# tahaspc82442/federated_multi_modal

Measured on AMD Instinct MI355X. Metric: images/sec/node (ViT-B/16 MaPLe fwd+bwd), higher is better.
Workload: dtype fp16; 1 GPU; c4: PatternNet-shape 38-class synthetic, J=9, batch=32 per client (configs[3]); clients=1, batch_per_client=32, global_batch=32, classes=38, prompt_depth=9, n_ctx=2, parallelism=one federated client per GPU x1, FedAvg all-reduce per round, round=512 local steps + 1 FedAvg, hipgraph=True

## Files before the change

### federated_multi_modal_amd/_lib.py

```python
from __future__ import annotations

import ctypes
import os
from pathlib import Path

_HERE = Path(__file__).resolve().parent
LIB_PATH = _HERE / "lib" / "libmapfed.so"

P, I, L, F = ctypes.c_void_p, ctypes.c_int, ctypes.c_int64, ctypes.c_float

SIGNATURES = {
    "mf_abi_version": [],
    "mf_gemm_nt": [P, L, P, L, P, L, I, I, I, P, P, P, L, I, I, P],
    "mf_gemm": [P, L, I, P, L, I, P, L, I, I, I, P, P, P, L, I, I, P],
    "mf_layernorm_fwd": [P, L, P, P, P, P, L, P, P, I, I, P],
    "mf_layernorm_bwd_blocks": [I],
    "mf_layernorm_bwd": [P, L, P, L, P, P, P, P, P, L, P, L, P, P, P, I, I, I, P],
    "mf_col_reduce_desc_bytes": [],
    "mf_col_reduce_batch": [P, I, I, P],
    "mf_attention_fwd": [P, L, P, L, P, I, I, I, I, I, P],
    "mf_attention_fwd_rows": [P, L, P, L, P, I, I, I, I, I, I, P],
    "mf_attention_bwd": [P, L, P, L, P, L, P, P, I, P, L, I, I, I, I, P],
    "mf_attention_bwd_rows": [P, L, P, L, P, L, P, I, P, L, I, I, I, I, I, P],
    "mf_qkv_attention_fwd": [P, L, I, P, P, P, L, P, L, P, I, I, I, I, I, P],
# ... 6 lines not shown
    "mf_transpose_f16": [P, L, P, L, I, I, P],
    "mf_colsum_blocks": [I],
    "mf_colsum_f16": [P, L, I, I, P, I, P, P],
    "mf_cast_f16_f32": [P, P, L, P],
    "mf_small_linear_fwd": [P, P, P, P, I, I, I, I, P],
    "mf_small_linear_bwd": [P, P, P, P, P, P, I, I, I, I, I, P],
    "mf_gemm_splitk_ws_floats": [I, I, I, I],
    "mf_small_linear_desc_bytes": [],
    "mf_small_linear_fwd_batch": [P, I, I, P],
    "mf_small_linear_bwd_batch": [P, I, I, I, I, P],
    "mf_clip_head_fwd": [P, P, I, I, I, P, P, P, P, P, P, P],
    "mf_clip_loss_fwd_bwd": [P, P, P, P, P, P, P, I, I, I, P, P, P, P, P, P, P, P, P],
    "mf_layernorm_bwd_inject": [P, L, P, L, P, P, P, P, L, P, L, P, I, I, P, I, I, I, P],
    "mf_layernorm_fwd_inject": [P, L, P, P, P, L, P, P, I, I, P, I, I, I, P],
    "mf_gemm_splitk": [P, L, I, P, L, I, P, L, I, I, I, P, L, I, I, P],
    "mf_clip_loss_soft_fwd_bwd": [P, P, P, P, P, P, P, I, I, I, P, P, P, P, P, P, P, P, P, P],
    "mf_argmax_correct": [P, I, I, P, P, P, P],
    "mf_optim_chunk_bytes": [],
    "mf_optim_chunk_elems": [],
    "mf_clip_grad_norm": [P, P, P, I, F, P, P, P],
    "mf_sgd_step": [P, P, P, L, I, P, P, P],
    "mf_optimizer_step": [P, P, P, L, P, P, P, L, P, I, F, P, P, P, P, P, P],
    "mf_sgd_prox_step": [P, P, P, P, L, I, P, P, P],
    "mf_optimizer_step_prox": [P, P, P, L, P, P, P, L, P, I, F, P, P, P, P, P, P, P, P],
    "mf_fedavg_pack_weighted": [P, L, P, L, P, F, P, P],
    "mf_fedavg_unpack_weighted": [P, P, L, P, L, P, P, P],
    "mf_fedavg_pack": [P, L, P, L, P, P, P],
    "mf_fedavg_unpack": [P, P, L, P, L, P, P, P],
    "mf_fedopt_step": [P, I, I, F, F, F, F, P, P, P, P, L, P, L, P, P, P],
    "mf_fedopt_deliver": [P, P, L, P, L, P, P, P],
# ... 55 lines not shown
```

### federated_multi_modal_amd/csrc/elementwise.hip

```cpp
#include "mf_common.h"

namespace {

template <typename TIn>
__global__ void im2col_kernel(const TIn* __restrict__ img, f16* __restrict__ out, int B, int R, int P) {
  const int G = R / P;
  const int K = 3 * P * P;
  const int chunks_per_row = K / 8;
  const int64_t t = (int64_t)blockIdx.x * blockDim.x + threadIdx.x;
  const int64_t total = (int64_t)B * G * G * chunks_per_row;
  if (t >= total) return;
  const int ch = t % chunks_per_row;
  const int64_t prow = t / chunks_per_row;
  const int b = prow / (G * G), pp = prow % (G * G);
  const int py = pp / G, px = pp % G;
  const int k = ch * 8;
  const int c = k / (P * P), kh = (k / P) % P, kw = k % P;
  const TIn* src = img + (((int64_t)b * 3 + c) * R + (py * P + kh)) * R + px * P + kw;
  f16x8 v;
  if constexpr (sizeof(TIn) == 4) {
    const f32x4 a = *(const f32x4*)src, d = *(const f32x4*)(src + 4);
#pragma unroll
    for (int e = 0; e < 4; ++e) {
      v[e] = (f16)a[e];
// ... 203 lines not shown
    return;
  }
  const int tx = t & 63, ty = t >> 6;
  for (int i = ty; i < 64; i += 4) {
    const int r = r0 + i, c = c0 + tx;
    tile[i][tx] = (r < R && c < C) ? in[(int64_t)r * ld_in + c] : (f16)0.f;
  }
  __syncthreads();
  for (int i = ty; i < 64; i += 4) {
    const int c = c0 + i, r = r0 + tx;
    if (c < C && r < R) out[(int64_t)c * ld_out + r] = tile[tx][i];
  }
}

constexpr int CS_ROWS = 64;
__global__ __launch_bounds__(256) void colsum_part_kernel(const f16* __restrict__ in, int64_t ld, int R, int C,
                                                          float* __restrict__ part) {
  __shared__ f32x4 red[4][64];
  const int lane = threadIdx.x & 63, w = threadIdx.x >> 6;
  const int c = blockIdx.x * 256 + lane * 4;
  const int r0 = blockIdx.y * CS_ROWS + w * 16;
  f32x4 s = {0.f, 0.f, 0.f, 0.f};
  if (c < C) {
#pragma unroll 4
    for (int r = r0; r < min(R, r0 + 16); ++r) {
      f16x4 v = *(const f16x4*)(in + (int64_t)r * ld + c);
#pragma unroll
      for (int e = 0; e < 4; ++e) s[e] += (float)v[e];
    }
  }
  red[w][lane] = s;
  __syncthreads();
  if (w == 0 && c < C) {
    f32x4 t = red[0][lane];
#pragma unroll
// ... 266 lines not shown
  MF_CHECK_LAUNCH();
  return 0;
}

extern "C" int mf_transpose_f16(const void* in, int64_t ld_in, void* out, int64_t ld_out, int R, int C,
                                void* stream) {
  if (R <= 0 || C <= 0) return 0;
  dim3 grid((C + 63) / 64, (R + 63) / 64);
  transpose_kernel<<<grid, 256, 0, (hipStream_t)stream>>>((const f16*)in, ld_in, (f16*)out, ld_out, R, C);
  MF_CHECK_LAUNCH();
  return 0;
}

extern "C" int mf_colsum_blocks(int R) { return (R + CS_ROWS - 1) / CS_ROWS; }

extern "C" int mf_colsum_f16(const void* in, int64_t ld, int R, int C, void* out, int out_f16, float* workspace,
                             void* stream) {
  if (R <= 0 || C <= 0) return 0;
  const int nb = mf_colsum_blocks(R);
  hipStream_t st = (hipStream_t)stream;
  if (C % 4 || ld % 4) return mf_set_error("mf_colsum_f16: C and ld must be multiples of 4", -1);
  dim3 grid((C + 255) / 256, nb);
  colsum_part_kernel<<<grid, 256, 0, st>>>((const f16*)in, ld, R, C, workspace);
  MF_CHECK_LAUNCH();
  if (out_f16)
    col_reduce_kernel<true><<<dim3((C + 63) / 64, 1), 1024, 0, st>>>(workspace, workspace, nb, C, C, out, out, 0);
  else
    col_reduce_kernel<false><<<dim3((C + 63) / 64, 1), 1024, 0, st>>>(workspace, workspace, nb, C, C, out, out, 0);
  MF_CHECK_LAUNCH();
  return 0;
}

extern "C" int mf_small_linear_fwd(const void* X, const void* W, const void* b, void* Y, int M, int I, int O,
                                   int is_f16, void* stream) {
  if (M <= 0) return 0;
  hipStream_t st = (hipStream_t)stream;
  const int64_t threads = (int64_t)M * O * 64;
  if (is_f16)
    small_linear_fwd_kernel<f16><<<nblk(threads), 256, 0, st>>>((const f16*)X, (const f16*)W, (const f16*)b, (f16*)Y,
                                                               M, I, O);
  else
    small_linear_fwd_kernel<float><<<nblk(threads), 256, 0, st>>>((const float*)X, (const float*)W,
                                                                  (const float*)b, (float*)Y, M, I, O);
  MF_CHECK_LAUNCH();
  return 0;
// ... 76 lines not shown
```

### federated_multi_modal_amd/csrc/gemm.hip

```cpp
#include <algorithm>
#include <cstdlib>
#include <type_traits>

#include "mf_common.h"

namespace {

enum Epi : int {
  EPI_NONE = 0,
  EPI_BIAS = 1,
  EPI_BIAS_RESID = 2,
  EPI_BIAS_GELU = 3,
  EPI_DGELU = 4,
  EPI_F32 = 5,
  EPI_RESID = 6,
};

struct GemmArgs {
  const f16* A;
  const f16* B;
  void* C;
  const f16* bias;
  const f16* aux_in;
  f16* aux_out;
  int64_t lda, ldb, ldc, ld_aux;
  int M, N, K;
  int vec8;
  int ksplit;
  int xb;
};

MF_DEV void st16_stream(f16* p, f16x8 v) { __builtin_nontemporal_store(v, (f16x8*)p); }

MF_DEV void tile_of(int p, int tiles_m, int tiles_n, int xb, int& mt, int& nt) {
  const int nb = 1 << xb, ma = 8 >> xb;
  int off = 0;
#pragma unroll 1
  for (int x = 0; x < 8; ++x) {
    const int ia = x >> xb, jb = x & (nb - 1);
    const int m_lo = tiles_m * ia / ma, m_hi = tiles_m * (ia + 1) / ma;
    const int n_lo = tiles_n * jb / nb, n_hi = tiles_n * (jb + 1) / nb;
    const int sz = (m_hi - m_lo) * (n_hi - n_lo);
    if (p < off + sz) {
      const int loc = p - off, w = n_hi - n_lo;
// ... 226 lines not shown
}

template <int A_INS, int B_INS>
MF_DEV void dma_stage(const f16* A, int a_bytes, const f16* B, int b_bytes, f16* la, f16* lb,
                      const int* a_voff, const int* a_dst, const int* b_voff, const int* b_dst, int a_k, int b_k) {
  const auto a_rsrc = __builtin_amdgcn_make_buffer_rsrc((void*)A, 0, a_bytes, 0x00020000);
  const auto b_rsrc = __builtin_amdgcn_make_buffer_rsrc((void*)B, 0, b_bytes, 0x00020000);
#pragma unroll
  for (int i = 0; i < A_INS; ++i)
    __builtin_amdgcn_raw_ptr_buffer_load_lds(a_rsrc, (lds_ptr_t)(la + a_dst[i]), 16, a_voff[i] + a_k, 0, 0, 0);
#pragma unroll
  for (int i = 0; i < B_INS; ++i)
    __builtin_amdgcn_raw_ptr_buffer_load_lds(b_rsrc, (lds_ptr_t)(lb + b_dst[i]), 16, b_voff[i] + b_k, 0, 0, 0);
}

template <int BM, int BN, int WM, int WN, int S, int EPI, bool TA = false, bool TB = false>
__global__ __launch_bounds__(WM * WN * 64) void gemm_nt_kernel(GemmArgs g0) {
  GemmArgs g = g0;
  constexpr int NW = WM * WN;
  constexpr int NT = NW * 64;
  constexpr int WTM = BM / WM, WTN = BN / WN;
  constexpr int TM = WTM / 16, TN = WTN / 16;
  constexpr int A_INS = BM / 8 / NW;
  constexpr int B_INS = BN / 8 / NW;
  static_assert(A_INS * 8 * NW == BM && B_INS * 8 * NW == BN, "tile / wave split");
  static_assert((!TA || BM == 64 || BM == 128) && (!TB || BN == 64 || BN == 128), "K-major image widths");
  constexpr int STAGE = (BM + BN) * BK;
  constexpr int LDS_ELEMS = S * STAGE > BM * (BN + 8) ? S * STAGE : BM * (BN + 8);
  __shared__ __attribute__((aligned(1024))) f16 lds[LDS_ELEMS];

  const int tid = threadIdx.x;
  const int lane = tid & 63;
  const int wid = __builtin_amdgcn_readfirstlane(tid >> 6);
  const int wave_m = wid / WN, wave_n = wid % WN;

  const int tiles_n = (g.N + BN - 1) / BN;
  const int tiles_m = (g.M + BM - 1) / BM;
  const bool legacy = g.ksplit > 0 && g.xb == 2;
  const int nwg = legacy ? tiles_m * tiles_n : gridDim.x;
  const int bid = legacy ? blockIdx.x % nwg : blockIdx.x;
  const int xcd = bid & 7, q = nwg >> 3, r = nwg & 7;
  const int wgid = (xcd < r ? xcd * (q + 1) : r * (q + 1) + (xcd - r) * q) + (bid >> 3);
  int mt, nt;
  if (g.ksplit > 0) {
    int z;
    if (legacy) {
      z = blockIdx.x / nwg;
      tile_of(wgid, tiles_m, tiles_n, 0, mt, nt);
    } else {
      split_tile_of(wgid, tiles_m, tiles_n, g.xb != 0, z, mt, nt);
    }
    const int k0 = z * g.ksplit;
    g.A += (int64_t)k0 * (TA ? g.lda : 1);
    g.B += (int64_t)k0 * (TB ? g.ldb : 1);
    g.K = min(g.ksplit, g.K - k0);
    g.C = (float*)g.C + (int64_t)z * g.M * g.ldc;
  } else {
    tile_of(wgid, tiles_m, tiles_n, g.xb, mt, nt);
  }
  const int m0 = mt * BM;
  const int n0 = nt * BN;

  const int a_bytes = (int)((TA ? (int64_t)(g.K - 1) * g.lda + g.M : (int64_t)(g.M - 1) * g.lda + g.K) * 2);
  const int b_bytes = (int)((TB ? (int64_t)(g.K - 1) * g.ldb + g.N : (int64_t)(g.N - 1) * g.ldb + g.K) * 2);
  int a_voff[A_INS], a_dst[A_INS], b_voff[B_INS], b_dst[B_INS];
#pragma unroll
  for (int i = 0; i < A_INS; ++i) dma_setup<TA, BM>(lane, wid, g.lda, m0, i, A_INS, a_voff[i], a_dst[i]);
// ... 2 lines not shown
  const int a_kstep = TA ? (int)(g.lda * 2) : 2, b_kstep = TB ? (int)(g.ldb * 2) : 2;
#define MF_STAGE(buf, k0)                                                                                     \
  dma_stage<A_INS, B_INS>(g.A, a_bytes, g.B, b_bytes, lds + (buf)*STAGE, lds + (buf)*STAGE + BM * BK, a_voff, a_dst, \
                          b_voff, b_dst, (k0)*a_kstep, (k0)*b_kstep)



  f32x4 acc[TM][TN];
#pragma unroll
  for (int i = 0; i < TM; ++i)
#pragma unroll
    for (int j = 0; j < TN; ++j) acc[i][j] = (f32x4){0.f, 0.f, 0.f, 0.f};

  MF_STAMP(0);
  const int nk = (g.K + BK - 1) / BK;
#pragma unroll
  for (int p = 0; p < S - 1; ++p)
    if (p < nk) MF_STAGE(p, p * BK);

  const int fr = lane & 15, fg = lane >> 4;
  for (int kt = 0; kt < nk; ++kt) {
    const int younger = min(S - 2, nk - 1 - kt);
    if constexpr (S >= 3) {
      if (younger >= 2) wait_vmcnt<2 * (A_INS + B_INS)>();
      else if (younger == 1) wait_vmcnt<A_INS + B_INS>();
      else wait_vmcnt<0>();
    } else {
      wait_vmcnt<0>();
    }
    __builtin_amdgcn_s_barrier();
    if (kt == 0) MF_STAMP(1);
    if (kt + S - 1 < nk) MF_STAGE((kt + S - 1) % S, (kt + S - 1) * BK);
    const f16* la = lds + (kt % S) * STAGE;
    const f16* lb = la + BM * BK;
    f16x8 af[2][TM], bf[2][TN];
#pragma unroll
    for (int s = 0; s < 2; ++s) {
#pragma unroll
      for (int i = 0; i < TM; ++i) {
        const int row = wave_m * WTM + i * 16 + fr;
        if constexpr (TA)
          af[s][i] = frag_t<BM>(la, 32 * s + 8 * fg, wave_m * WTM + i * 16, fr);
        else
          af[s][i] = *(const f16x8*)(la + row * BK + swz(row, 4 * s + fg) * 8);
      }
#pragma unroll
      for (int j = 0; j < TN; ++j) {
        const int row = wave_n * WTN + j * 16 + fr;
        if constexpr (TB)
          bf[s][j] = frag_t<BN>(lb, 32 * s + 8 * fg, wave_n * WTN + j * 16, fr);
        else
          bf[s][j] = *(const f16x8*)(lb + row * BK + swz(row, 4 * s + fg) * 8);
      }
    }
#pragma unroll
    for (int s = 0; s < 2; ++s)
#pragma unroll
      for (int i = 0; i < TM; ++i)
#pragma unroll
        for (int j = 0; j < TN; ++j)
          acc[i][j] = __builtin_amdgcn_mfma_f32_16x16x32_f16(bf[s][j], af[s][i], acc[i][j], 0, 0, 0);
  }

#undef MF_STAGE
  MF_STAMP(2);
  __syncthreads();
  epilogue_store<BM, BN, NT, TM, TN, EPI>(g, lds, acc, m0, n0, wave_m * WTM, wave_n * WTN, tid, fr, fg);
  MF_STAMP(3);
}

template <int BM, int BN, int WM, int WN, int EPI>
__global__ __launch_bounds__(512) void gemm8_kernel(GemmArgs g) {
  constexpr int NT = 512;
  static_assert(WM * WN == 8, "8 waves");
  constexpr int WTM = BM / WM, WTN = BN / WN;
  constexpr int QM = WTM / 2;
// ... 904 lines not shown
    case 21: return K < 128 ? launch_tile<128, 128, 2, 2, 2>(a, epilogue, st) : launch_tile8<256, 128, 2, 4>(a, epilogue, st);
    case 22: return K < 128 ? launch_tile<128, 128, 2, 2, 2>(a, epilogue, st) : launch_tile8<256, 256, 2, 4>(a, epilogue, st);
    case 40: return K < 128 ? launch_tile<128, 128, 2, 2, 2>(a, epilogue, st) : launch_tile8f(a, epilogue, st);
    case 41: return K < 128 ? launch_tile<128, 128, 2, 2, 2>(a, epilogue, st) : launch_tile8p(a, epilogue, st);
    case 50: return launch_small_m(a, epilogue, st);
    default: return mf_set_error("mf_gemm: bad tile id", -2);
  }
}

extern "C" int mf_gemm_nt(const void* A, int64_t lda, const void* B, int64_t ldb, void* C, int64_t ldc, int M,
                          int N, int K, const void* bias, const void* aux_in, void* aux_out, int64_t ld_aux,
                          int epilogue, int tile, void* stream) {
  return mf_gemm(A, lda, 0, B, ldb, 0, C, ldc, M, N, K, bias, aux_in, aux_out, ld_aux, epilogue, tile, stream);
}

extern "C" int mf_gemm_splitk(const void* A, int64_t lda, int a_kmajor, const void* B, int64_t ldb, int b_kmajor,
                              void* C, int64_t ldc, int M, int N, int K, float* ws, int64_t ws_floats, int splits,
                              int out_f16, void* stream) {
  if (M <= 0 || N <= 0) return 0;
  const bool both_k = a_kmajor && b_kmajor;
  if (K <= 0 || (!both_k && (K % BK) != 0))
    return mf_set_error("mf_gemm_splitk: K must be a positive multiple of 64 unless both operands are K-major", -1);
  if ((N % 8) != 0 || (lda % 8) || (ldb % 8) || (ldc % 4)) return mf_set_error("mf_gemm_splitk: alignment", -1);
  if ((a_kmajor && (M % 8 || lda < M)) || (b_kmajor && (N % 8 || ldb < N)) || (!a_kmajor && lda < K) ||
      (!b_kmajor && ldb < K))
    return mf_set_error("mf_gemm_splitk: K-major operands need rows % 8 == 0 and ld >= rows; row-major ld >= K", -1);
  if ((uintptr_t)A % 16 || (uintptr_t)B % 16 || (uintptr_t)ws % 16 || (uintptr_t)C % 16)
    return mf_set_error("mf_gemm_splitk: pointers must be 16-byte aligned", -1);
  const int64_t tiles = (int64_t)((M + 127) / 128) * ((N + 127) / 128);
  if (splits <= 0) splits = splitk_auto(tiles);
  int ks = (int)((((int64_t)K + splits - 1) / splits + BK - 1) / BK * BK);
  if (ks < BK) ks = BK;
  splits = (K + ks - 1) / ks;
  if ((int64_t)splits * M * N > ws_floats) return mf_set_error("mf_gemm_splitk: workspace too small", -1);
  hipStream_t st = (hipStream_t)stream;
  const bool slice_major = tiles >= 96;
  GemmArgs a{(const f16*)A, (const f16*)B, ws, nullptr, nullptr, nullptr, lda, ldb, (int64_t)N, 0, M, N, K, 1, ks,
             slice_major ? ((N > M) ? 1 : 0) : 2};
  int rc;
  if (a_kmajor && b_kmajor) rc = launch_tile<128, 128, 2, 2, 2, true, true>(a, EPI_F32, st);
  else if (a_kmajor) rc = launch_tile<128, 128, 2, 2, 2, true, false>(a, EPI_F32, st);
  else if (b_kmajor) rc = launch_tile<128, 128, 2, 2, 2, false, true>(a, EPI_F32, st);
  else rc = launch_tile<128, 128, 2, 2, 2>(a, EPI_F32, st);
  if (rc) return rc;
  const int64_t nq = (int64_t)M * (N / 4);
  splitk_reduce_kernel<<<(unsigned)((nq + 255) / 256), 256, 0, st>>>(ws, splits, M, N, C, ldc, out_f16);
  MF_CHECK_LAUNCH();
  return 0;
}

extern "C" int mf_gemm_splitk_ws_floats(int M, int N, int K, int splits) {
  const int64_t tiles = (int64_t)((M + 127) / 128) * ((N + 127) / 128);
  if (splits <= 0) splits = splitk_auto(tiles);
  int ks = (int)((((int64_t)K + splits - 1) / splits + BK - 1) / BK * BK);
  if (ks < BK) ks = BK;
  splits = (K + ks - 1) / ks;
  const int64_t n = (int64_t)splits * M * N;
  return n > 0x7fffffff ? -1 : (int)n;
}
```

### federated_multi_modal_amd/csrc/layernorm.hip

```cpp
#include <cstdlib>

#include "mf_common.h"

#pragma clang fp contract(off)

namespace {

constexpr int LN_WAVES = 4;
constexpr int LN_ROWS_PER_BLOCK = 16;

template <int D>
__global__ __launch_bounds__(256) void ln_fwd_kernel(const f16* __restrict__ x, int64_t ldx,
                                                    const int* __restrict__ ridx, const float* __restrict__ gamma,
                                                    const float* __restrict__ beta, f16* __restrict__ y,
                                                    int64_t ldy, float* __restrict__ mean_out,
                                                    float* __restrict__ rstd_out, int rows) {
  constexpr int CH = D / 256;
  const int lane = threadIdx.x & 63;
  const int row = blockIdx.x * LN_WAVES + (threadIdx.x >> 6);
  if (row >= rows) return;
  const int src = ridx ? ridx[row] : row;
  const f16* xr = x + (int64_t)src * ldx;
  float v[CH * 4];
  float s = 0.f;
// ... 415 lines not shown
  else
    ln_bwd_kernel<512><<<nblk, 256, 0, st>>>((const f16*)dy, lddy, (const f16*)x, ldx, row_index, gamma, mean, rstd,
                                             (const f16*)dres, ldres, (f16*)dx, lddx, dg_part, db_part, rows);
  MF_CHECK_LAUNCH();
  if (!dgamma && !dbeta) return 0;
  if (!dgamma || !dbeta) return mf_set_error("mf_layernorm_bwd: dgamma and dbeta go together", -1);
  col_reduce_kernel<false><<<dim3((D + 63) / 64, 2), 1024, 0, st>>>(dg_part, db_part, nblk, D, D, dgamma, dbeta,
                                                                    accumulate);
  MF_CHECK_LAUNCH();
  return 0;
}

namespace {
struct ColReduceDesc {
  const float* part;
  float* out;
  int nblk, C, accumulate, pad;
};
__global__ __launch_bounds__(1024) void col_reduce_batch_kernel(const ColReduceDesc* __restrict__ descs) {
  __shared__ float red[16][65];
  const ColReduceDesc d = descs[blockIdx.y];
  if ((int)blockIdx.x * 64 >= d.C) return;
  const int lane = threadIdx.x & 63, g = threadIdx.x >> 6;
  const int c = blockIdx.x * 64 + lane;
  float s0 = 0.f, s1 = 0.f, s2 = 0.f, s3 = 0.f;
  if (c < d.C) {
    int b = g;
    for (; b + 48 < d.nblk; b += 64) {
      s0 += d.part[(int64_t)b * d.C + c];
      s1 += d.part[(int64_t)(b + 16) * d.C + c];
      s2 += d.part[(int64_t)(b + 32) * d.C + c];
      s3 += d.part[(int64_t)(b + 48) * d.C + c];
    }
    for (; b < d.nblk; b += 16) s0 += d.part[(int64_t)b * d.C + c];
  }
  red[g][lane] = (s0 + s1) + (s2 + s3);
  __syncthreads();
  if (g == 0 && c < d.C) {
    float s = 0.f;
#pragma unroll
    for (int k = 0; k < 16; ++k) s += red[k][lane];
    d.out[c] = d.accumulate ? d.out[c] + s : s;
  }
}
}

extern "C" int mf_col_reduce_desc_bytes(void) { return (int)sizeof(ColReduceDesc); }

extern "C" int mf_col_reduce_batch(const void* descs, int n, int max_cols, void* stream) {
  if (n <= 0) return 0;
  col_reduce_batch_kernel<<<dim3((max_cols + 63) / 64, n), 1024, 0, (hipStream_t)stream>>>(
      (const ColReduceDesc*)descs);
  MF_CHECK_LAUNCH();
  return 0;
}

extern "C" int mf_prompt_inject_fwd_ld(void* x, int64_t ldx, const float* prompt, int N, int L, int row0, int nrows,
// ... 90 lines not shown
```

### federated_multi_modal_amd/engine.py

```python
from __future__ import annotations

import math
import os
from dataclasses import dataclass, field
from typing import Dict, List, Optional, Tuple

import numpy as np
import torch

from . import ops
from . import synthetic as syn
from .tokenizer import get_tokenizer

F16, F32 = torch.float16, torch.float32
N_CTX = 2


@dataclass
class EngineConfig:
    batch: int
    classnames: List[str]
    prompt_depth: int = 9
    seed: int = 0
    n_ctx: int = N_CTX
# ... 208 lines not shown
        self.G = e(R, 4 * D)
        self.dX = e(R, D)
        self.dX2 = e(R, D) if any(self.grow) else None
        self.dX1 = e(R, D)
        self.dO = e(R, D)
        self.dH = e(R, D)
        self.dQKV = e(R, 3 * D)
        self.dF = e(R, 4 * D)
        self.attn_ws = e(N * H * max(self.Ls), dt=F32)
        sel = eng.cfg.fused_qkv_attn
        if sel not in ("side", "none", "both", "vision", "text"):
            raise ValueError(f"EngineConfig.fused_qkv_attn: {sel!r}")
        self.fused_qkv_attn = sel == "both" or sel == ("vision" if name == "image_encoder" else "text")
        self.tile = 0
        self.lnb = ops.LNGradBatch(dev)
        self.cs_ws = e(ops.colsum_ws_floats(R if self.live is None else N * self.live[1], 4 * D), dt=F32)
        shapes = ((3 * D, D), (D, D), (4 * D, D), (D, 4 * D))
        Rl = Rs[-1] if self.live is None else N * self.live[1]
        ws = {s: ops.gemm_splitk_ws_floats(s[0], s[1], Rl) for s in shapes}
        self.dw_split = {s for s in shapes if ws[s] > s[0] * s[1]}
        self.dw_ws = e(max(ws[s] for s in self.dw_split), dt=F32) if self.dw_split else None
        self.full_dy = self.full_x = None
        if self.live is not None:
            z = lambda: torch.zeros(Rl, 4 * D, device=dev, dtype=F16)
            self.full_dy, self.full_x = z(), z()

    def _alloc_forward_only(self, e, R, N, H, D, layers):
        xb = (e(R, D), e(R, D))
        self.X = [xb[i % 2] for i in range(layers + 1)]
        self.Y = self.X[1:]
        one = lambda *s, dt=F16: [e(*s, dt=dt)] * layers
        self.QKV, self.O, self.X1, self.Fp = one(R, 3 * D), one(R, D), one(R, D), one(R, 4 * D)
        self.LSE = one(N * H * self.L, dt=F32)
        self.mean1, self.rstd1, self.mean2, self.rstd2 = (one(R, dt=F32) for _ in range(4))
        self.H1, self.H2, self.G = e(R, D), e(R, D), e(R, 4 * D)
        self.dX = self.dX2 = self.dX1 = self.dO = self.dH = self.dQKV = self.dF = self.attn_ws = None
        self.fused_qkv_attn = self.e.cfg.fused_qkv_attn in ("both", "vision" if self.name == "image_encoder"
                                                             else "text")
        self.tile = 0
        self.lnb = self.cs_ws = self.dw_ws = None
        self.dw_split = set()

    def p(self, i: int, key: str) -> torch.Tensor:
        return self.e.P[f"{self.name}.transformer.resblocks.{i}.{key}"]

    def wt(self, i: int, key: str) -> torch.Tensor:
        return self.e.WT[f"{self.name}.transformer.resblocks.{i}.{key}"]

    def g(self, i: int, key: str) -> torch.Tensor:
        return self.e.G[f"{self.name}.transformer.resblocks.{i}.{key}"]

    def forward(self, deep_prompts: List[torch.Tensor], cap: Optional[torch.Tensor] = None):
        N, D, H = self.N, self.D, self.H
        self._cls_fwd = self.train_cls_rows and self._cls_pass
        for i in range(self.layers):
# ... 68 lines not shown
        h2 = self.cls_H2[::L]
        ops.layernorm_fwd(x1, self.p(i, "ln_2.weight"), self.p(i, "ln_2.bias"), h2, self.mean2[i][:N],
                          self.rstd2[i][:N])
        g = self.cls_G[::L]
        ops.gemm_nt(h2, self.p(i, "mlp.c_fc.weight"), g, bias=self.p(i, "mlp.c_fc.bias"), aux_out=self.Fp[i][::L],
                    epilogue=ops.EPI_BIAS_GELU, tile=self.tile)
        ops.gemm_nt(g, self.p(i, "mlp.c_proj.weight"), self.Y[i][::L], bias=self.p(i, "mlp.c_proj.bias"), aux_in=x1,
                    epilogue=ops.EPI_BIAS_RESID, tile=self.tile)

    def _last_block_bwd_cls_rows(self, i: int, L: int, R: int):
        N, H = self.N, self.H
        dX = self.dX[:R]
        dXc, dFc, dHc = dX[::L], self.cls_dF[:R][::L], self.dH[:R][::L]
        ops.gemm_nt(dXc, self.wt(i, "mlp.c_proj.weight"), dFc, aux_in=self.Fp[i][::L], epilogue=ops.EPI_DGELU,
                    tile=self.tile)
        self._dw(dX, self.cls_G[:R], self.g(i, "mlp.c_proj.weight"), self.g(i, "mlp.c_proj.bias"))
        ops.gemm_nt(dFc, self.wt(i, "mlp.c_fc.weight"), dHc, epilogue=ops.EPI_NONE, tile=self.tile)
        self._dw(self.cls_dF[:R], self.cls_H2[:R], self.g(i, "mlp.c_fc.weight"), self.g(i, "mlp.c_fc.bias"))
        self.lnb.bwd(dHc, self.X1[i][::L], self.p(i, "ln_2.weight"), self.mean2[i][:N], self.rstd2[i][:N], dXc,
                     self.g(i, "ln_2.weight"), self.g(i, "ln_2.bias"), dres=dXc, live=(1, L))
        ops.gemm_nt(dXc, self.wt(i, "attn.out_proj.weight"), self.dO[:R][::L], epilogue=ops.EPI_NONE, tile=self.tile)
        self._dw(dX, self.O[i], self.g(i, "attn.out_proj.weight"), self.g(i, "attn.out_proj.bias"))
        ops.attention_bwd_rows(self.QKV[i], self.O[i], self.dO[:R], self.LSE[i], N, L, H, self.causal, 1,
                               dqkv=self.dQKV[:R])

    def _dw(self, dY: torch.Tensor, Xin: torch.Tensor, dW: torch.Tensor, db: torch.Tensor):
        if self.live is not None:
            Ll, Lf = self.live
            for src, full in ((dY, self.full_dy), (Xin, self.full_x)):
                assert src.shape[0] == self.N * Ll and src.shape[1] <= full.shape[1] and full.shape[0] == self.N * Lf
            dY = ops.seq_scatter(dY, self.full_dy[:, :dY.shape[1]], self.N, Ll, Lf)[:self.N * Lf]
            Xin = ops.seq_scatter(Xin, self.full_x[:, :Xin.shape[1]], self.N, Ll, Lf)[:self.N * Lf]
        if tuple(dW.shape) in self.dw_split:
            ops.gemm_splitk(dY, Xin, dW, self.dw_ws, a_kmajor=True, b_kmajor=True)
        else:
            ops.gemm(dY, Xin, dW, epilogue=ops.EPI_NONE, a_kmajor=True, b_kmajor=True)
        ops.colsum(dY, db, self.cs_ws)

    def backward(self, n_prompted: int, prompt_grads: List[torch.Tensor]):
        if self.inference:
            raise RuntimeError("backward on a forward-only (EngineConfig.inference) engine")
        N, D, H = self.N, self.D, self.H
        last = self.layers - 1
        for i in reversed(range(self.layers)):
            L, R = self.Ls[i], self.Rs[i]
            dX = self.dX[:R]
            dF, dH, dO, dQKV = self.dF[:R], self.dH[:R], self.dO[:R], self.dQKV[:R]
            trainable_w = i == last
            if trainable_w and self._cls_fwd:
                self._last_block_bwd_cls_rows(i, L, R)
            else:
                ops.gemm_nt(dX, self.wt(i, "mlp.c_proj.weight"), dF, aux_in=self.Fp[i], epilogue=ops.EPI_DGELU,
# ... 580 lines not shown
```

### federated_multi_modal_amd/ops.py

```python
from __future__ import annotations

import ctypes
import os
from typing import Optional

import torch

from ._lib import call

EPI_NONE, EPI_BIAS, EPI_BIAS_RESID, EPI_BIAS_GELU, EPI_DGELU, EPI_F32, EPI_RESID = range(7)


class KernelProbe:

    def __init__(self, kinds="gemm"):
        self.kinds = {kinds} if isinstance(kinds, str) else set(kinds)
        self.kind = next(iter(self.kinds)) if len(self.kinds) == 1 else None
        self.records = []

    def wants(self, kind: str) -> bool:
        return kind in self.kinds

    def around(self, flops: float, nbytes: float, key: str = "gemm", meta=None):
        s = torch.cuda.Event(enable_timing=True)
# ... 112 lines not shown
    call("mf_gemm", _p(A), _ld(A), int(a_kmajor), _p(B), _ld(B), int(b_kmajor), _p(C), _ld(C), M, N, K, _p(bias),
         _p(aux_in), _p(aux_out), ld_aux, epilogue, tile, _s())
    if ev is not None:
        ev.record()
    return C



def gemm_splitk_ws_floats(M: int, N: int, K: int, splits: int = 0) -> int:
    n = call("mf_gemm_splitk_ws_floats", M, N, K, splits)
    if n < 0:
        raise ValueError("split-K workspace exceeds 2^31 floats")
    return n


def gemm_splitk(A, B, C, ws, splits=0, a_kmajor=False, b_kmajor=False):
    M, Ka = (A.shape[1], A.shape[0]) if a_kmajor else A.shape
    N, Kb = (B.shape[1], B.shape[0]) if b_kmajor else B.shape
    assert Ka == Kb, (A.shape, a_kmajor, B.shape, b_kmajor)
    K = Ka
    assert ws.dtype == torch.float32 and C.dtype in (torch.float16, torch.float32)
    ev = None
    if _PROBE is not None and _PROBE.wants("gemm"):
        ev = _PROBE.around(2.0 * M * N * K, _gemm_bytes(M, N, K, C), _gkey(), (M, N, K, "splitk"))
    call("mf_gemm_splitk", _p(A), _ld(A), int(a_kmajor), _p(B), _ld(B), int(b_kmajor), _p(C), _ld(C), M, N, K,
         _p(ws), ws.numel(), splits, int(C.dtype == torch.float16), _s())
    if ev is not None:
        ev.record()
    return C


def layernorm_fwd(x, gamma, beta, y=None, mean=None, rstd=None, row_index=None):
    rows = row_index.numel() if row_index is not None else x.shape[0]
    D = x.shape[1]
    if y is None:
        y = torch.empty(rows, D, device=x.device, dtype=torch.float16)
    if mean is None:
        mean = torch.empty(rows, device=x.device, dtype=torch.float32)
    if rstd is None:
        rstd = torch.empty(rows, device=x.device, dtype=torch.float32)
    ev = _hbm(f"layernorm_fwd/D{D}", rows * D * 4.0 + rows * 8.0)
# ... 119 lines not shown
        if ikey not in self.ws:
            n = rows // L
            part = torch.empty(n * nrows * D, device=self.device, dtype=torch.float32)
            self.ws[ikey] = part
            self.descs.append((part.data_ptr(), prompt_grad.data_ptr(), n, nrows * D))
            self.max_cols = max(self.max_cols, nrows * D)
            self.dev_descs = None
        ev = _hbm(f"layernorm_bwd/D{D}", rows * D * (6.0 + (2.0 if dres is not None else 0.0)) + rows * 8.0
                  + (self.ws[key].numel() + self.ws[ikey].numel()) * 4.0)
        call("mf_layernorm_bwd_inject", _p(dy), _ld(dy), _p(x), _ld(x), _p(gamma), _p(mean), _p(rstd), _p(dres),
             _ld(dres) if dres is not None else 0, _p(dx), _ld(dx), _p(self.ws[key]), rows, D, _p(self.ws[ikey]), L,
             row0, nrows, _s())
        _rec(ev)
        return dx

    def finish(self):
        if not self.descs:
            return
        if self.dev_descs is None:
            import numpy as np
            assert call("mf_col_reduce_desc_bytes") == 32
            arr = np.zeros(len(self.descs), dtype=np.dtype([("part", np.uint64), ("out", np.uint64),
                                                            ("nblk", np.int32), ("C", np.int32),
                                                            ("acc", np.int32), ("pad", np.int32)]))
            for i, (pp, op, nb, c) in enumerate(self.descs):
                arr[i] = (pp, op, nb, c, 0, 0)
            self.dev_descs = torch.from_numpy(arr.view(np.uint8)).to(self.device)
        call("mf_col_reduce_batch", _p(self.dev_descs), len(self.descs), self.max_cols, _s())


def attention_fwd(qkv, N, L, H, causal, out=None, lse=None, ld_lse=None):
    D = H * 64
    if out is None:
        out = torch.empty(N * L, D, device=qkv.device, dtype=torch.float16)
    if ld_lse is None:
        ld_lse = L
    if lse is None:
        lse = torch.empty(N * H * ld_lse, device=qkv.device, dtype=torch.float32)
    ev = None
    if _PROBE is not None and _PROBE.wants("attention"):
        pairs = L * (L + 1) / 2 if causal else L * L
# ... 126 lines not shown
    assert tokens.dtype == torch.int32 and table.dtype == torch.float32 and w.dtype == torch.float16
    call("mf_caption_pool", _p(tokens), B, T, _p(table), table.shape[0], _p(w), table.shape[1], _p(pooled), _s())
    return pooled


def transpose(inp, out):
    R, C = inp.shape
    call("mf_transpose_f16", _p(inp), _ld(inp), _p(out), _ld(out), R, C, _s())
    return out


def colsum_ws_floats(R: int, C: int) -> int:
    return call("mf_colsum_blocks", R) * C


def colsum(inp, out, workspace=None):
    R, C = inp.shape
    if workspace is None:
        workspace = torch.empty(colsum_ws_floats(R, C), device=inp.device, dtype=torch.float32)
    call("mf_colsum_f16", _p(inp), _ld(inp), R, C, _p(out), int(out.dtype == torch.float16), _p(workspace), _s())
    return out


def small_linear_fwd(X, W, b, Y):
    M, I = X.shape
    O = W.shape[0]
    call("mf_small_linear_fwd", _p(X), _p(W), _p(b), _p(Y), M, I, O, int(X.dtype == torch.float16), _s())
    return Y


class SmallLinearBatch:

    def __init__(self, device, entries):
        import numpy as np
        assert call("mf_small_linear_desc_bytes") == 88
# ... 249 lines not shown
```

### include/mapfed.h

```cpp
#ifndef MAPFED_H_
#define MAPFED_H_
#include <stdint.h>

#ifdef __cplusplus
extern "C" {
#endif

const char* mf_last_error(void);
int mf_abi_version(void);

int mf_gemm_nt(const void* A, int64_t lda, const void* B, int64_t ldb, void* C, int64_t ldc, int M, int N, int K,
               const void* bias, const void* aux_in, void* aux_out, int64_t ld_aux, int epilogue, int tile,
               void* stream);
int mf_gemm(const void* A, int64_t lda, int a_kmajor, const void* B, int64_t ldb, int b_kmajor, void* C, int64_t ldc,
            int M, int N, int K, const void* bias, const void* aux_in, void* aux_out, int64_t ld_aux, int epilogue,
            int tile, void* stream);
int mf_gemm_splitk(const void* A, int64_t lda, int a_kmajor, const void* B, int64_t ldb, int b_kmajor, void* C,
                   int64_t ldc, int M, int N, int K, float* ws, int64_t ws_floats, int splits, int out_f16,
                   void* stream);
int mf_gemm_splitk_ws_floats(int M, int N, int K, int splits);

int mf_layernorm_fwd(const void* x, int64_t ldx, const int* row_index, const float* gamma, const float* beta,
                     void* y, int64_t ldy, float* mean, float* rstd, int rows, int D, void* stream);
int mf_layernorm_fwd_inject(void* x, int64_t ldx, const float* gamma, const float* beta, void* y, int64_t ldy,
                            float* mean, float* rstd, int rows, int D, const float* prompt, int L, int row0,
                            int nrows, void* stream);
int mf_layernorm_bwd_blocks(int rows);
int mf_layernorm_bwd(const void* dy, int64_t lddy, const void* x, int64_t ldx, const int* row_index,
                     const float* gamma, const float* mean, const float* rstd, const void* dres, int64_t ldres,
                     void* dx, int64_t lddx, float* dgamma, float* dbeta, float* workspace, int rows, int D,
                     int accumulate, void* stream);

int mf_layernorm_bwd_inject(const void* dy, int64_t lddy, const void* x, int64_t ldx, const float* gamma,
                            const float* mean, const float* rstd, const void* dres, int64_t ldres, void* dx,
                            int64_t lddx, float* workspace, int rows, int D, float* inj_part, int L, int row0,
// ... 29 lines not shown
                     int L, int n_ctx, int D, void* stream);
int mf_prompt_inject_fwd(void* x, const float* prompt, int N, int L, int row0, int nrows, int D, void* stream);
int mf_prompt_inject_bwd(void* dx, int N, int L, int row0, int nrows, int D, void* out, int out_f16, int accumulate,
                         int zero_rows, void* stream);

int mf_seq_grow(const void* src, void* dst, const void* cap, const float* prompt, int N, int Lp, int ncap, int n_ctx,
                int D, void* stream);
int mf_seq_grow_bwd(const void* ddst, void* dsrc, int N, int Lp, int ncap, int n_ctx, int D, void* stream);
int mf_caption_pool(const int* tokens, int B, int T, const float* table, int vocab, const void* w, int D,
                    void* pooled, void* stream);
int mf_transpose_f16(const void* in, int64_t ld_in, void* out, int64_t ld_out, int R, int C, void* stream);
int mf_seq_scatter(const void* src, int64_t ld_src, void* dst, int64_t ld_dst, int N, int L_live, int L_full, int C,
                   void* stream);
int mf_colsum_blocks(int R);
int mf_colsum_f16(const void* in, int64_t ld, int R, int C, void* out, int out_f16, float* workspace, void* stream);
int mf_cast_f16_f32(const void* in, float* out, int64_t n, void* stream);

int mf_small_linear_fwd(const void* X, const void* W, const void* b, void* Y, int M, int I, int O, int is_f16,
                        void* stream);
int mf_small_linear_bwd(const void* dY, const void* X, const void* W, void* dX, void* dW, void* db, int M, int I,
                        int O, int is_f16, int accumulate_dx, void* stream);

int mf_small_linear_desc_bytes(void);
int mf_small_linear_fwd_batch(const void* descs, int n, int max_mo, void* stream);
int mf_small_linear_bwd_batch(const void* descs, int n, int max_m, int max_i, int max_oi, void* stream);

int mf_clip_head_fwd(const void* img, const void* txt, int B, int K, int D, const float* logit_scale, void* img_n,
                     void* txt_n, float* norms, void* mm, void* logits, void* stream);
int mf_clip_loss_fwd_bwd(const void* img, const void* txt, const void* img_n, const void* txt_n, const float* norms,
                         const void* logits, const int64_t* label, int B, int K, int D, const float* logit_scale,
// ... 52 lines not shown
```

Before: 5785 images/s.

## Skip dead sequence rows in last-layer weight-gradient split-K GEMM and bias colsum

In the last encoder layer only the CLS row of each sequence carries gradient, so the weight-gradient split-K GEMM and the bias column sum now skip K-tiles and row blocks that fall entirely outside the live prefix (L_live=1 of L_full). The GEMM gets a LIVE template path that stages only live K-tiles. The bias colsum is routed through the batched LN-grad column-reduce, which gains an fp16 output flag, removing one reduce launch per call. With L_live=1 and BK-sized tiles spanning several sequences, few tiles may actually be skippable, and the GEMM pipeline becomes more irregular.

Measured after the change: 5847 images/s, median of 6. +1.1%, better.

```diff
diff --git a/federated_multi_modal_amd/_lib.py b/federated_multi_modal_amd/_lib.py
--- a/federated_multi_modal_amd/_lib.py
+++ b/federated_multi_modal_amd/_lib.py
@@ -44,6 +44,8 @@
     "mf_layernorm_bwd_inject": [P, L, P, L, P, P, P, P, L, P, L, P, I, I, P, I, I, I, P],
     "mf_layernorm_fwd_inject": [P, L, P, P, P, L, P, P, I, I, P, I, I, I, P],
     "mf_gemm_splitk": [P, L, I, P, L, I, P, L, I, I, I, P, L, I, I, P],
+    "mf_gemm_splitk_live": [P, L, I, P, L, I, P, L, I, I, I, P, L, I, I, I, I, I, P],
+    "mf_colsum_f16_live": [P, L, I, I, P, I, P, I, I, P],
     "mf_clip_loss_soft_fwd_bwd": [P, P, P, P, P, P, P, I, I, I, P, P, P, P, P, P, P, P, P, P],
     "mf_argmax_correct": [P, I, I, P, P, P, P],
     "mf_optim_chunk_bytes": [],
diff --git a/federated_multi_modal_amd/csrc/elementwise.hip b/federated_multi_modal_amd/csrc/elementwise.hip
--- a/federated_multi_modal_amd/csrc/elementwise.hip
+++ b/federated_multi_modal_amd/csrc/elementwise.hip
@@ -241,11 +241,19 @@
 }
 
 constexpr int CS_ROWS = 64;
+template <bool LIVE>
 __global__ __launch_bounds__(256) void colsum_part_kernel(const f16* __restrict__ in, int64_t ld, int R, int C,
-                                                          float* __restrict__ part) {
+                                                          float* __restrict__ part, int l_live, int l_full) {
   __shared__ f32x4 red[4][64];
   const int lane = threadIdx.x & 63, w = threadIdx.x >> 6;
   const int c = blockIdx.x * 256 + lane * 4;
+  if constexpr (LIVE) {
+    const int rc = blockIdx.y * CS_ROWS, s = rc % l_full, nxt = rc + (l_full - s);
+    if (s >= l_live && (nxt >= rc + CS_ROWS || nxt >= R)) {
+      if (w == 0 && c < C) *(f32x4*)(part + (int64_t)blockIdx.y * C + c) = f32x4{0.f, 0.f, 0.f, 0.f};
+      return;
+    }
+  }
   const int r0 = blockIdx.y * CS_ROWS + w * 16;
   f32x4 s = {0.f, 0.f, 0.f, 0.f};
   if (c < C) {
@@ -542,21 +550,35 @@
 
 extern "C" int mf_colsum_blocks(int R) { return (R + CS_ROWS - 1) / CS_ROWS; }
 
-extern "C" int mf_colsum_f16(const void* in, int64_t ld, int R, int C, void* out, int out_f16, float* workspace,
-                             void* stream) {
+static int colsum_run(const void* in, int64_t ld, int R, int C, void* out, int out_f16, float* workspace, int l_live,
+                      int l_full, void* stream) {
   if (R <= 0 || C <= 0) return 0;
   const int nb = mf_colsum_blocks(R);
   hipStream_t st = (hipStream_t)stream;
   if (C % 4 || ld % 4) return mf_set_error("mf_colsum_f16: C and ld must be multiples of 4", -1);
   dim3 grid((C + 255) / 256, nb);
-  colsum_part_kernel<<<grid, 256, 0, st>>>((const f16*)in, ld, R, C, workspace);
-  MF_CHECK_LAUNCH();
+  if (l_full > 0) colsum_part_kernel<true><<<grid, 256, 0, st>>>((const f16*)in, ld, R, C, workspace, l_live, l_full);
+  else colsum_part_kernel<false><<<grid, 256, 0, st>>>((const f16*)in, ld, R, C, workspace, 0, 0);
+  MF_CHECK_LAUNCH();
+  if (!out) return 0;
   if (out_f16)
     col_reduce_kernel<true><<<dim3((C + 63) / 64, 1), 1024, 0, st>>>(workspace, workspace, nb, C, C, out, out, 0);
   else
     col_reduce_kernel<false><<<dim3((C + 63) / 64, 1), 1024, 0, st>>>(workspace, workspace, nb, C, C, out, out, 0);
   MF_CHECK_LAUNCH();
   return 0;
+}
+
+extern "C" int mf_colsum_f16(const void* in, int64_t ld, int R, int C, void* out, int out_f16, float* workspace,
+                             void* stream) {
+  return colsum_run(in, ld, R, C, out, out_f16, workspace, 0, 0, stream);
+}
+
+extern "C" int mf_colsum_f16_live(const void* in, int64_t ld, int R, int C, void* out, int out_f16, float* workspace,
+                                  int L_live, int L_full, void* stream) {
+  if (L_full <= 0 || L_live <= 0 || L_live > L_full || R % L_full != 0)
+    return mf_set_error("mf_colsum_f16_live: needs 0 < L_live <= L_full and R % L_full == 0", -1);
+  return colsum_run(in, ld, R, C, out, out_f16, workspace, L_live, L_full, stream);
 }
 
 extern "C" int mf_small_linear_fwd(const void* X, const void* W, const void* b, void* Y, int M, int I, int O,
diff --git a/federated_multi_modal_amd/csrc/gemm.hip b/federated_multi_modal_amd/csrc/gemm.hip
--- a/federated_multi_modal_amd/csrc/gemm.hip
+++ b/federated_multi_modal_amd/csrc/gemm.hip
@@ -28,6 +28,10 @@
   int vec8;
   int ksplit;
   int xb;
+};
+
+struct GemmArgsLive : GemmArgs {
+  int l_full, l_live, m_live;
 };
 
 MF_DEV void st16_stream(f16* p, f16x8 v) { __builtin_nontemporal_store(v, (f16x8*)p); }
@@ -284,8 +288,9 @@
     __builtin_amdgcn_raw_ptr_buffer_load_lds(b_rsrc, (lds_ptr_t)(lb + b_dst[i]), 16, b_voff[i] + b_k, 0, 0, 0);
 }
 
-template <int BM, int BN, int WM, int WN, int S, int EPI, bool TA = false, bool TB = false>
-__global__ __launch_bounds__(WM * WN * 64) void gemm_nt_kernel(GemmArgs g0) {
+template <int BM, int BN, int WM, int WN, int S, int EPI, bool TA = false, bool TB = false, bool LIVE = false>
+__global__ __launch_bounds__(WM * WN * 64) void gemm_nt_kernel(std::conditional_t<LIVE, GemmArgsLive, GemmArgs> g0) {
+  static_assert(!LIVE || (TA && TB && EPI == EPI_F32), "the live K loop is the split-K weight-gradient tile's");
   GemmArgs g = g0;
   constexpr int NW = WM * WN;
   constexpr int NT = NW * 64;
@@ -312,6 +317,8 @@
   const int xcd = bid & 7, q = nwg >> 3, r = nwg & 7;
   const int wgid = (xcd < r ? xcd * (q + 1) : r * (q + 1) + (xcd - r) * q) + (bid >> 3);
   int mt, nt;
+  const int k_all = g.K;
+  int kt0 = 0;
   if (g.ksplit > 0) {
     int z;
     if (legacy) {
@@ -321,6 +328,7 @@
       split_tile_of(wgid, tiles_m, tiles_n, g.xb != 0, z, mt, nt);
     }
     const int k0 = z * g.ksplit;
+    kt0 = k0 / BK;
     g.A += (int64_t)k0 * (TA ? g.lda : 1);
     g.B += (int64_t)k0 * (TB ? g.ldb : 1);
     g.K = min(g.ksplit, g.K - k0);
@@ -353,24 +361,15 @@
 
   MF_STAMP(0);
   const int nk = (g.K + BK - 1) / BK;
-#pragma unroll
-  for (int p = 0; p < S - 1; ++p)
-    if (p < nk) MF_STAGE(p, p * BK);
+  if constexpr (!LIVE) {
+#pragma unroll
+    for (int p = 0; p < S - 1; ++p)
+      if (p < nk) MF_STAGE(p, p * BK);
+  }
 
   const int fr = lane & 15, fg = lane >> 4;
-  for (int kt = 0; kt < nk; ++kt) {
-    const int younger = min(S - 2, nk - 1 - kt);
-    if constexpr (S >= 3) {
-      if (younger >= 2) wait_vmcnt<2 * (A_INS + B_INS)>();
-      else if (younger == 1) wait_vmcnt<A_INS + B_INS>();
-      else wait_vmcnt<0>();
-    } else {
-      wait_vmcnt<0>();
-    }
-    __builtin_amdgcn_s_barrier();
-    if (kt == 0) MF_STAMP(1);
-    if (kt + S - 1 < nk) MF_STAGE((kt + S - 1) % S, (kt + S - 1) * BK);
-    const f16* la = lds + (kt % S) * STAGE;
+  auto consume = [&](int buf) {
+    const f16* la = lds + buf * STAGE;
     const f16* lb = la + BM * BK;
     f16x8 af[2][TM], bf[2][TN];
 #pragma unroll
@@ -399,6 +398,57 @@
 #pragma unroll
         for (int j = 0; j < TN; ++j)
           acc[i][j] = __builtin_amdgcn_mfma_f32_16x16x32_f16(bf[s][j], af[s][i], acc[i][j], 0, 0, 0);
+  };
+  if constexpr (LIVE) {
+    const bool dense = min(m0 + BM, g.M) > g0.m_live;
+    auto next_live = [&](int t) {
+      if (dense || t >= nk) return t;
+      const int r = (kt0 + t) * BK;
+      const int s = r % g0.l_full;
+      if (s < g0.l_live) return t;
+      const int nxt = r + (g0.l_full - s);
+      return nxt >= k_all ? nk : nxt / BK - kt0;
+    };
+    int cur = next_live(0), issued = 0;
+#pragma unroll
+    for (int p = 0; p < S - 1; ++p)
+      if (cur < nk) {
+        MF_STAGE(p, cur * BK);
+        ++issued;
+        cur = next_live(cur + 1);
+      }
+    for (int i = 0; i < issued; ++i) {
+      const int younger = issued - 1 - i;
+      if constexpr (S >= 3) {
+        if (younger >= 2) wait_vmcnt<2 * (A_INS + B_INS)>();
+        else if (younger == 1) wait_vmcnt<A_INS + B_INS>();
+        else wait_vmcnt<0>();
+      } else {
+        wait_vmcnt<0>();
+      }
+      __builtin_amdgcn_s_barrier();
+      if (cur < nk) {
+        MF_STAGE(issued % S, cur * BK);
+        ++issued;
+        cur = next_live(cur + 1);
+      }
+      consume(i % S);
+    }
+  } else {
+    for (int kt = 0; kt < nk; ++kt) {
+      const int younger = min(S - 2, nk - 1 - kt);
+      if constexpr (S >= 3) {
+        if (younger >= 2) wait_vmcnt<2 * (A_INS + B_INS)>();
+        else if (younger == 1) wait_vmcnt<A_INS + B_INS>();
+        else wait_vmcnt<0>();
+      } else {
+        wait_vmcnt<0>();
+      }
+      __builtin_amdgcn_s_barrier();
+      if (kt == 0) MF_STAMP(1);
+      if (kt + S - 1 < nk) MF_STAGE((kt + S - 1) % S, (kt + S - 1) * BK);
+      consume(kt % S);
+    }
   }
 
 #undef MF_STAGE
@@ -1333,9 +1383,9 @@
   return mf_gemm(A, lda, 0, B, ldb, 0, C, ldc, M, N, K, bias, aux_in, aux_out, ld_aux, epilogue, tile, stream);
 }
 
-extern "C" int mf_gemm_splitk(const void* A, int64_t lda, int a_kmajor, const void* B, int64_t ldb, int b_kmajor,
-                              void* C, int64_t ldc, int M, int N, int K, float* ws, int64_t ws_floats, int splits,
-                              int out_f16, void* stream) {
+static int splitk_run(const void* A, int64_t lda, int a_kmajor, const void* B, int64_t ldb, int b_kmajor, void* C,
+                      int64_t ldc, int M, int N, int K, float* ws, int64_t ws_floats, int splits, int out_f16,
+                      int l_live, int l_full, int m_live, void* stream) {
   if (M <= 0 || N <= 0) return 0;
   const bool both_k = a_kmajor && b_kmajor;
   if (K <= 0 || (!both_k && (K % BK) != 0))
@@ -1356,8 +1406,12 @@
   const bool slice_major = tiles >= 96;
   GemmArgs a{(const f16*)A, (const f16*)B, ws, nullptr, nullptr, nullptr, lda, ldb, (int64_t)N, 0, M, N, K, 1, ks,
              slice_major ? ((N > M) ? 1 : 0) : 2};
-  int rc;
-  if (a_kmajor && b_kmajor) rc = launch_tile<128, 128, 2, 2, 2, true, true>(a, EPI_F32, st);
+  int rc = 0;
+  if (l_full > 0) {
+    const GemmArgsLive al{a, l_full, l_live, m_live};
+    gemm_nt_kernel<128, 128, 2, 2, 2, EPI_F32, true, true, true><<<dim3(tiles * splits), dim3(256), 0, st>>>(al);
+    MF_CHECK_LAUNCH();
+  } else if (a_kmajor && b_kmajor) rc = launch_tile<128, 128, 2, 2, 2, true, true>(a, EPI_F32, st);
   else if (a_kmajor) rc = launch_tile<128, 128, 2, 2, 2, true, false>(a, EPI_F32, st);
   else if (b_kmajor) rc = launch_tile<128, 128, 2, 2, 2, false, true>(a, EPI_F32, st);
   else rc = launch_tile<128, 128, 2, 2, 2>(a, EPI_F32, st);
@@ -1368,6 +1422,25 @@
   return 0;
 }
 
+extern "C" int mf_gemm_splitk(const void* A, int64_t lda, int a_kmajor, const void* B, int64_t ldb, int b_kmajor,
+                              void* C, int64_t ldc, int M, int N, int K, float* ws, int64_t ws_floats, int splits,
+                              int out_f16, void* stream) {
+  return splitk_run(A, lda, a_kmajor, B, ldb, b_kmajor, C, ldc, M, N, K, ws, ws_floats, splits, out_f16, 0, 0, 0,
+                    stream);
+}
+
+extern "C" int mf_gemm_splitk_live(const void* A, int64_t lda, int a_kmajor, const void* B, int64_t ldb,
+                                   int b_kmajor, void* C, int64_t ldc, int M, int N, int K, float* ws,
+                                   int64_t ws_floats, int splits, int out_f16, int L_live, int L_full, int m_live,
+                                   void* stream) {
+  if (!a_kmajor || !b_kmajor) return mf_set_error("mf_gemm_splitk_live: both operands must be K-major", -1);
+  if (L_full <= 0 || L_live <= 0 || L_live > L_full || K % L_full != 0)
+    return mf_set_error("mf_gemm_splitk_live: needs 0 < L_live <= L_full and K % L_full == 0", -1);
+  if (m_live < 0) return mf_set_error("mf_gemm_splitk_live: m_live < 0", -1);
+  return splitk_run(A, lda, 1, B, ldb, 1, C, ldc, M, N, K, ws, ws_floats, splits, out_f16, L_live, L_full,
+                    m_live > M ? M : m_live, stream);
+}
+
 extern "C" int mf_gemm_splitk_ws_floats(int M, int N, int K, int splits) {
   const int64_t tiles = (int64_t)((M + 127) / 128) * ((N + 127) / 128);
   if (splits <= 0) splits = splitk_auto(tiles);
diff --git a/federated_multi_modal_amd/csrc/layernorm.hip b/federated_multi_modal_amd/csrc/layernorm.hip
--- a/federated_multi_modal_amd/csrc/layernorm.hip
+++ b/federated_multi_modal_amd/csrc/layernorm.hip
@@ -453,8 +453,8 @@
 namespace {
 struct ColReduceDesc {
   const float* part;
-  float* out;
-  int nblk, C, accumulate, pad;
+  void* out;
+  int nblk, C, accumulate, out_f16;
 };
 __global__ __launch_bounds__(1024) void col_reduce_batch_kernel(const ColReduceDesc* __restrict__ descs) {
   __shared__ float red[16][65];
@@ -479,7 +479,13 @@
     float s = 0.f;
 #pragma unroll
     for (int k = 0; k < 16; ++k) s += red[k][lane];
-    d.out[c] = d.accumulate ? d.out[c] + s : s;
+    if (d.out_f16) {
+      f16* o = (f16*)d.out + c;
+      *o = d.accumulate ? (f16)((float)*o + s) : (f16)s;
+    } else {
+      float* o = (float*)d.out + c;
+      *o = d.accumulate ? *o + s : s;
+    }
   }
 }
 }
diff --git a/federated_multi_modal_amd/engine.py b/federated_multi_modal_amd/engine.py
--- a/federated_multi_modal_amd/engine.py
+++ b/federated_multi_modal_amd/engine.py
@@ -246,7 +246,6 @@
         self.fused_qkv_attn = sel == "both" or sel == ("vision" if name == "image_encoder" else "text")
         self.tile = 0
         self.lnb = ops.LNGradBatch(dev)
-        self.cs_ws = e(ops.colsum_ws_floats(R if self.live is None else N * self.live[1], 4 * D), dt=F32)
         shapes = ((3 * D, D), (D, D), (4 * D, D), (D, 4 * D))
         Rl = Rs[-1] if self.live is None else N * self.live[1]
         ws = {s: ops.gemm_splitk_ws_floats(s[0], s[1], Rl) for s in shapes}
@@ -270,7 +269,7 @@
         self.fused_qkv_attn = self.e.cfg.fused_qkv_attn in ("both", "vision" if self.name == "image_encoder"
                                                              else "text")
         self.tile = 0
-        self.lnb = self.cs_ws = self.dw_ws = None
+        self.lnb = self.dw_ws = None
         self.dw_split = set()
 
     def p(self, i: int, key: str) -> torch.Tensor:
@@ -369,17 +368,18 @@
         dXc, dFc, dHc = dX[::L], self.cls_dF[:R][::L], self.dH[:R][::L]
         ops.gemm_nt(dXc, self.wt(i, "mlp.c_proj.weight"), dFc, aux_in=self.Fp[i][::L], epilogue=ops.EPI_DGELU,
                     tile=self.tile)
-        self._dw(dX, self.cls_G[:R], self.g(i, "mlp.c_proj.weight"), self.g(i, "mlp.c_proj.bias"))
+        self._dw(dX, self.cls_G[:R], self.g(i, "mlp.c_proj.weight"), self.g(i, "mlp.c_proj.bias"), dead=(1, L))
         ops.gemm_nt(dFc, self.wt(i, "mlp.c_fc.weight"), dHc, epilogue=ops.EPI_NONE, tile=self.tile)
-        self._dw(self.cls_dF[:R], self.cls_H2[:R], self.g(i, "mlp.c_fc.weight"), self.g(i, "mlp.c_fc.bias"))
+        self._dw(self.cls_dF[:R], self.cls_H2[:R], self.g(i, "mlp.c_fc.weight"), self.g(i, "mlp.c_fc.bias"),
+                 dead=(1, L))
         self.lnb.bwd(dHc, self.X1[i][::L], self.p(i, "ln_2.weight"), self.mean2[i][:N], self.rstd2[i][:N], dXc,
                      self.g(i, "ln_2.weight"), self.g(i, "ln_2.bias"), dres=dXc, live=(1, L))
         ops.gemm_nt(dXc, self.wt(i, "attn.out_proj.weight"), self.dO[:R][::L], epilogue=ops.EPI_NONE, tile=self.tile)
-        self._dw(dX, self.O[i], self.g(i, "attn.out_proj.weight"), self.g(i, "attn.out_proj.bias"))
+        self._dw(dX, self.O[i], self.g(i, "attn.out_proj.weight"), self.g(i, "attn.out_proj.bias"), dead=(1, L))
         ops.attention_bwd_rows(self.QKV[i], self.O[i], self.dO[:R], self.LSE[i], N, L, H, self.causal, 1,
                                dqkv=self.dQKV[:R])
 
-    def _dw(self, dY: torch.Tensor, Xin: torch.Tensor, dW: torch.Tensor, db: torch.Tensor):
+    def _dw(self, dY: torch.Tensor, Xin: torch.Tensor, dW: torch.Tensor, db: torch.Tensor, dead=None):
         if self.live is not None:
             Ll, Lf = self.live
             for src, full in ((dY, self.full_dy), (Xin, self.full_x)):
@@ -387,10 +387,10 @@
             dY = ops.seq_scatter(dY, self.full_dy[:, :dY.shape[1]], self.N, Ll, Lf)[:self.N * Lf]
             Xin = ops.seq_scatter(Xin, self.full_x[:, :Xin.shape[1]], self.N, Ll, Lf)[:self.N * Lf]
         if tuple(dW.shape) in self.dw_split:
-            ops.gemm_splitk(dY, Xin, dW, self.dw_ws, a_kmajor=True, b_kmajor=True)
+            ops.gemm_splitk(dY, Xin, dW, self.dw_ws, a_kmajor=True, b_kmajor=True, live=dead)
         else:
             ops.gemm(dY, Xin, dW, epilogue=ops.EPI_NONE, a_kmajor=True, b_kmajor=True)
-        ops.colsum(dY, db, self.cs_ws)
+        self.lnb.colsum(dY, db, live=dead)
 
     def backward(self, n_prompted: int, prompt_grads: List[torch.Tensor]):
         if self.inference:
diff --git a/federated_multi_modal_amd/ops.py b/federated_multi_modal_amd/ops.py
--- a/federated_multi_modal_amd/ops.py
+++ b/federated_multi_modal_amd/ops.py
@@ -150,7 +150,7 @@
     return n
 
 
-def gemm_splitk(A, B, C, ws, splits=0, a_kmajor=False, b_kmajor=False):
+def gemm_splitk(A, B, C, ws, splits=0, a_kmajor=False, b_kmajor=False, live=None, m_live=None):
     M, Ka = (A.shape[1], A.shape[0]) if a_kmajor else A.shape
     N, Kb = (B.shape[1], B.shape[0]) if b_kmajor else B.shape
     assert Ka == Kb, (A.shape, a_kmajor, B.shape, b_kmajor)
@@ -159,8 +159,13 @@
     ev = None
     if _PROBE is not None and _PROBE.wants("gemm"):
         ev = _PROBE.around(2.0 * M * N * K, _gemm_bytes(M, N, K, C), _gkey(), (M, N, K, "splitk"))
-    call("mf_gemm_splitk", _p(A), _ld(A), int(a_kmajor), _p(B), _ld(B), int(b_kmajor), _p(C), _ld(C), M, N, K,
-         _p(ws), ws.numel(), splits, int(C.dtype == torch.float16), _s())
+    if live is not None:
+        call("mf_gemm_splitk_live", _p(A), _ld(A), int(a_kmajor), _p(B), _ld(B), int(b_kmajor), _p(C), _ld(C), M, N,
+             K, _p(ws), ws.numel(), splits, int(C.dtype == torch.float16), live[0], live[1],
+             M if m_live is None else m_live, _s())
+    else:
+        call("mf_gemm_splitk", _p(A), _ld(A), int(a_kmajor), _p(B), _ld(B), int(b_kmajor), _p(C), _ld(C), M, N, K,
+             _p(ws), ws.numel(), splits, int(C.dtype == torch.float16), _s())
     if ev is not None:
         ev.record()
     return C
@@ -310,6 +315,19 @@
         _rec(ev)
         return dx
 
+    def colsum(self, dy, db, live=None):
+        R, C = dy.shape
+        key = ("db", db.data_ptr())
+        nblk = call("mf_colsum_blocks", R)
+        if key not in self.ws:
+            part = torch.empty(nblk * C, device=self.device, dtype=torch.float32)
+            self.ws[key] = part
+            self.descs.append((part.data_ptr(), db.data_ptr(), nblk, C, int(db.dtype == torch.float16)))
+            self.max_cols = max(self.max_cols, C)
+            self.dev_descs = None
+        assert self.ws[key].numel() == nblk * C and db.numel() == C
+        colsum(dy, None, self.ws[key], live=live)
+
     def finish(self):
         if not self.descs:
             return
@@ -318,9 +336,9 @@
             assert call("mf_col_reduce_desc_bytes") == 32
             arr = np.zeros(len(self.descs), dtype=np.dtype([("part", np.uint64), ("out", np.uint64),
                                                             ("nblk", np.int32), ("C", np.int32),
-                                                            ("acc", np.int32), ("pad", np.int32)]))
-            for i, (pp, op, nb, c) in enumerate(self.descs):
-                arr[i] = (pp, op, nb, c, 0, 0)
+                                                            ("acc", np.int32), ("out_f16", np.int32)]))
+            for i, (pp, op, nb, c, *f16) in enumerate(self.descs):
+                arr[i] = (pp, op, nb, c, 0, f16[0] if f16 else 0)
             self.dev_descs = torch.from_numpy(arr.view(np.uint8)).to(self.device)
         call("mf_col_reduce_batch", _p(self.dev_descs), len(self.descs), self.max_cols, _s())
 
@@ -477,11 +495,15 @@
     return call("mf_colsum_blocks", R) * C
 
 
-def colsum(inp, out, workspace=None):
+def colsum(inp, out, workspace=None, live=None):
     R, C = inp.shape
     if workspace is None:
         workspace = torch.empty(colsum_ws_floats(R, C), device=inp.device, dtype=torch.float32)
-    call("mf_colsum_f16", _p(inp), _ld(inp), R, C, _p(out), int(out.dtype == torch.float16), _p(workspace), _s())
+    f16 = int(out is not None and out.dtype == torch.float16)
+    if live is not None:
+        call("mf_colsum_f16_live", _p(inp), _ld(inp), R, C, _p(out), f16, _p(workspace), live[0], live[1], _s())
+    else:
+        call("mf_colsum_f16", _p(inp), _ld(inp), R, C, _p(out), f16, _p(workspace), _s())
     return out
 
 
diff --git a/include/mapfed.h b/include/mapfed.h
--- a/include/mapfed.h
+++ b/include/mapfed.h
@@ -19,6 +19,9 @@
                    int64_t ldc, int M, int N, int K, float* ws, int64_t ws_floats, int splits, int out_f16,
                    void* stream);
 int mf_gemm_splitk_ws_floats(int M, int N, int K, int splits);
+int mf_gemm_splitk_live(const void* A, int64_t lda, int a_kmajor, const void* B, int64_t ldb, int b_kmajor, void* C,
+                        int64_t ldc, int M, int N, int K, float* ws, int64_t ws_floats, int splits, int out_f16,
+                        int L_live, int L_full, int m_live, void* stream);
 
 int mf_layernorm_fwd(const void* x, int64_t ldx, const int* row_index, const float* gamma, const float* beta,
                      void* y, int64_t ldy, float* mean, float* rstd, int rows, int D, void* stream);
@@ -78,6 +81,8 @@
                    void* stream);
 int mf_colsum_blocks(int R);
 int mf_colsum_f16(const void* in, int64_t ld, int R, int C, void* out, int out_f16, float* workspace, void* stream);
+int mf_colsum_f16_live(const void* in, int64_t ld, int R, int C, void* out, int out_f16, float* workspace,
+                       int L_live, int L_full, void* stream);
 int mf_cast_f16_f32(const void* in, float* out, int64_t n, void* stream);
 
 int mf_small_linear_fwd(const void* X, const void* W, const void* b, void* Y, int M, int I, int O, int is_f16,
```
